# Electron-Labs/eth-lc-plonky2

Measured on AMD Instinct MI355X. Metric: lc_proofs_per_hour, higher is better.
Workload: dtype u64

## Files before the change

eth-lc-plonky2_amd/csrc/kernels_hash.hip:

```cpp
#include "internal.hpp"
#include "poseidon.hpp"

namespace lcp2 {

constexpr int HASH_THREADS = 256;

__global__ __launch_bounds__(HASH_THREADS) void k_poseidon_permute_batch(const u64 *__restrict__ in, u64 *__restrict__ out,
                                                                          size_t count, const u64 *__restrict__ rc) {
  size_t i = (size_t)blockIdx.x * blockDim.x + threadIdx.x;
  if (i >= count) return;
  u64 s[12];
#pragma unroll
  for (int j = 0; j < 12; j++) s[j] = gl_canon(in[i * 12 + j]);
  pos_permute(s, rc);
#pragma unroll
  for (int j = 0; j < 12; j++) out[i * 12 + j] = s[j];
}

__global__ __launch_bounds__(HASH_THREADS) void k_field_op(const u64 *__restrict__ a, const u64 *__restrict__ b, u64 *__restrict__ out,
                                                            size_t count, u32 op) {
  size_t i = (size_t)blockIdx.x * blockDim.x + threadIdx.x;
  if (i >= count) return;
#if defined(__HIP_DEVICE_COMPILE__)
  const u64 x = a[i], y = b ? b[i] : 0;
  u64 r = 0;
  switch (op) {
    case LCP2_FIELD_MUL: r = gl_mul(x, y); break;
    case LCP2_FIELD_POW7: { u32 r0 = (u32)x, r1 = (u32)(x >> 32); pos_sbox_h(r0, r1); r = gl_canon(((u64)r1 << 32) | r0); break; }
    case LCP2_FIELD_ADD: r = gl_add(gl_canon(x), gl_canon(y)); break;
    case LCP2_FIELD_SUB: r = gl_sub(gl_canon(x), gl_canon(y)); break;
    case LCP2_FIELD_CANON: r = gl_canon(x); break;
    case LCP2_FIELD_ADD_LAZY: r = gl_canon(gl_add_nc(x, gl_canon(y))); break;
    case LCP2_FIELD_SUB_LAZY: r = gl_canon(gl_sub_nc(x, gl_canon(y))); break;
    case LCP2_FIELD_SHL + 1: r = gl_shl<12>(gl_canon(x)); break;
    case LCP2_FIELD_SHL + 2: r = gl_shl<24>(gl_canon(x)); break;
    case LCP2_FIELD_SHL + 3: r = gl_shl<36>(gl_canon(x)); break;
    case LCP2_FIELD_SHL + 4: r = gl_shl<48>(gl_canon(x)); break;
    case LCP2_FIELD_SHL + 5: r = gl_shl<60>(gl_canon(x)); break;
    case LCP2_FIELD_SHL + 6: r = gl_shl<72>(gl_canon(x)); break;
    case LCP2_FIELD_SHL + 7: r = gl_shl<84>(gl_canon(x)); break;
    case LCP2_FIELD_SHL + 8: r = gl_canon(gl_shl_nc<32>(x)); break;
    case LCP2_FIELD_SHL + 9: r = gl_canon(gl_mul_u32_nc(x, (u32)y)); break;
  }
  out[i] = r;
#endif
}

__global__ __launch_bounds__(HASH_THREADS, 5) void k_hash_leaves(const u64 *__restrict__ data, u64 leaf_stride, u64 col_stride,
                                                               u32 leaf_len, u64 nleaves, u64 *__restrict__ digests,
                                                               const u64 *__restrict__ rc) {
  u64 i = (u64)blockIdx.x * blockDim.x + threadIdx.x;
  if (i >= nleaves) return;
  const u64 *row = data + i * leaf_stride;
  u64 s[12];
#pragma unroll
  for (int j = 0; j < 12; j++) s[j] = 0;
  if (leaf_len <= 4) {
    for (u32 c = 0; c < leaf_len; c++) s[c] = gl_canon(row[c * col_stride]);
  } else {
    for (u32 c0 = 0; c0 < leaf_len; c0 += 8) {
      if (c0 + 8 <= leaf_len) {
#pragma unroll
        for (int j = 0; j < 8; j++) s[j] = gl_canon(row[(u64)(c0 + j) * col_stride]);
      } else {
#pragma unroll
        for (int j = 0; j < 8; j++)
          if (c0 + j < leaf_len) s[j] = gl_canon(row[(u64)(c0 + j) * col_stride]);
      }
      pos_permute(s, rc);
    }
  }
  ulonglong2 *d = (ulonglong2 *)(digests + 4 * i);
  d[0] = make_ulonglong2(s[0], s[1]);
  d[1] = make_ulonglong2(s[2], s[3]);
}

__global__ __launch_bounds__(HASH_THREADS, 5) void k_hash_leaves_absorb(const u64 *__restrict__ data, u64 col_stride, u32 ncols, u64 nleaves,
                                                                      u64 *__restrict__ state, u32 first, u32 last, u64 *__restrict__ digests,
                                                                      const u64 *__restrict__ rc) {
  u64 i = (u64)blockIdx.x * blockDim.x + threadIdx.x;
  if (i >= nleaves) return;
  const u64 *row = data + i;
  u64 s[12];
#pragma unroll
  for (int j = 0; j < 12; j++) s[j] = first ? 0 : state[(u64)j * nleaves + i];
  for (u32 c0 = 0; c0 < ncols; c0 += 8) {
    if (c0 + 8 <= ncols) {
#pragma unroll
      for (int j = 0; j < 8; j++) s[j] = gl_canon(row[(u64)(c0 + j) * col_stride]);
    } else {
#pragma unroll
      for (int j = 0; j < 8; j++)
        if (c0 + j < ncols) s[j] = gl_canon(row[(u64)(c0 + j) * col_stride]);
    }
    pos_permute(s, rc);
  }
  if (last) {
    ulonglong2 *d = (ulonglong2 *)(digests + 4 * i);
    d[0] = make_ulonglong2(s[0], s[1]);
    d[1] = make_ulonglong2(s[2], s[3]);
  } else {
#pragma unroll
    for (int j = 0; j < 12; j++) state[(u64)j * nleaves + i] = s[j];
  }
}

__global__ __launch_bounds__(HASH_THREADS, 5) void k_hash_ext_leaves(const u64 *__restrict__ p0, const u64 *__restrict__ p1, u32 arity,
                                                                   u64 nleaves, u64 *__restrict__ digests,
                                                                   const u64 *__restrict__ rc) {
  u64 i = (u64)blockIdx.x * blockDim.x + threadIdx.x;
  if (i >= nleaves) return;
  const u64 *a = p0 + i * arity, *b = p1 + i * arity;
  u64 s[12];
#pragma unroll
  for (int j = 0; j < 12; j++) s[j] = 0;
  u32 len = 2 * arity;
  if (len <= 4) {
    for (u32 e = 0; e < arity; e++) { s[2 * e] = a[e]; s[2 * e + 1] = b[e]; }
  } else {
    for (u32 e0 = 0; e0 < arity; e0 += 4) {
#pragma unroll
      for (int j = 0; j < 4; j++)
        if (e0 + j < arity) { s[2 * j] = a[e0 + j]; s[2 * j + 1] = b[e0 + j]; }
      pos_permute(s, rc);
    }
  }
  ulonglong2 *d = (ulonglong2 *)(digests + 4 * i);
  d[0] = make_ulonglong2(s[0], s[1]);
  d[1] = make_ulonglong2(s[2], s[3]);
}

__global__ __launch_bounds__(HASH_THREADS) void k_merkle_level(const u64 *__restrict__ children, u64 *__restrict__ parents,
                                                                u64 nparents, const u64 *__restrict__ rc) {
  u64 i = (u64)blockIdx.x * blockDim.x + threadIdx.x;
  if (i >= nparents) return;
  const ulonglong2 *c = (const ulonglong2 *)(children + 8 * i);
  ulonglong2 c0 = c[0], c1 = c[1], c2 = c[2], c3 = c[3];
  u64 s[12] = {c0.x, c0.y, c1.x, c1.y, c2.x, c2.y, c3.x, c3.y, 0, 0, 0, 0};
  pos_permute(s, rc);
  ulonglong2 *d = (ulonglong2 *)(parents + 4 * i);
  d[0] = make_ulonglong2(s[0], s[1]);
  d[1] = make_ulonglong2(s[2], s[3]);
}

constexpr int COOP_THREADS = 256;
__device__ __forceinline__ void coop_load_rc(u64 *rcs, const u64 *__restrict__ rc) {
  for (u32 i = threadIdx.x; i < POS_ROUNDS * POS_W; i += COOP_THREADS) rcs[i] = rc[i];
  __syncthreads();
}
__global__ __launch_bounds__(COOP_THREADS) void k_merkle_level_coop(const u64 *__restrict__ children, u64 *__restrict__ parents,
                                                                      u64 nparents, const u64 *__restrict__ rc) {
  __shared__ u64 rcs[POS_ROUNDS * POS_W];
  coop_load_rc(rcs, rc);
  const u64 t = (u64)blockIdx.x * COOP_THREADS + threadIdx.x, node = t >> 4;
  const u32 j = (u32)t & 15;
  const bool live = node < nparents;
  const u64 nd = live ? node : 0;
  const u64 v = j < 8 ? children[8 * nd + j] : 0;
  const u64 r = pos_permute_coop(v, j, rcs);
  if (live && j < 4) parents[4 * nd + j] = r;
}
__global__ __launch_bounds__(COOP_THREADS) void k_hash_ext_leaves_coop(const u64 *__restrict__ p0, const u64 *__restrict__ p1, u32 arity,
                                                                         u64 nleaves, u64 *__restrict__ digests, const u64 *__restrict__ rc) {
  __shared__ u64 rcs[POS_ROUNDS * POS_W];
  coop_load_rc(rcs, rc);
  const u64 t = (u64)blockIdx.x * COOP_THREADS + threadIdx.x, leaf = t >> 4;
  const u32 j = (u32)t & 15;
  const bool live = leaf < nleaves;
  const u64 lf = live ? leaf : 0;
  const u64 *src = ((j & 1) ? p1 : p0) + lf * arity + (j >> 1);
  u64 v = 0;
  for (u32 e0 = 0; e0 < arity; e0 += 4) {
    if (j < 8 && e0 + (j >> 1) < arity) v = src[e0];
    v = pos_permute_coop(v, j, rcs);
  }
  if (live && j < 4) digests[4 * lf + j] = v;
}

__device__ __constant__ uint32_t SHA_K[64] = {
    0x428a2f98, 0x71374491, 0xb5c0fbcf, 0xe9b5dba5, 0x3956c25b, 0x59f111f1, 0x923f82a4, 0xab1c5ed5, 0xd807aa98, 0x12835b01,
    0x243185be, 0x550c7dc3, 0x72be5d74, 0x80deb1fe, 0x9bdc06a7, 0xc19bf174, 0xe49b69c1, 0xefbe4786, 0x0fc19dc6, 0x240ca1cc,
    0x2de92c6f, 0x4a7484aa, 0x5cb0a9dc, 0x76f988da, 0x983e5152, 0xa831c66d, 0xb00327c8, 0xbf597fc7, 0xc6e00bf3, 0xd5a79147,
    0x06ca6351, 0x14292967, 0x27b70a85, 0x2e1b2138, 0x4d2c6dfc, 0x53380d13, 0x650a7354, 0x766a0abb, 0x81c2c92e, 0x92722c85,
    0xa2bfe8a1, 0xa81a664b, 0xc24b8b70, 0xc76c51a3, 0xd192e819, 0xd6990624, 0xf40e3585, 0x106aa070, 0x19a4c116, 0x1e376c08,
    0x2748774c, 0x34b0bcb5, 0x391c0cb3, 0x4ed8aa4a, 0x5b9cca4f, 0x682e6ff3, 0x748f82ee, 0x78a5636f, 0x84c87814, 0x8cc70208,
    0x90befffa, 0xa4506ceb, 0xbef9a3f7, 0xc67178f2};

__device__ __forceinline__ uint32_t rotr(uint32_t x, int r) { return __builtin_rotateright32(x, r); }

__device__ __forceinline__ void sha256_compress(uint32_t st[8], uint32_t w[16], uint32_t *trace) {
  uint32_t a = st[0], b = st[1], c = st[2], d = st[3], e = st[4], f = st[5], g = st[6], h = st[7];
#pragma unroll 1
  for (int i = 0; i < 64; i++) {
    uint32_t wi;
    if (i < 16) {
      wi = w[i & 15];
    } else {
      uint32_t w15 = w[(i - 15) & 15], w2 = w[(i - 2) & 15];
      uint32_t s0 = rotr(w15, 7) ^ rotr(w15, 18) ^ (w15 >> 3);
      uint32_t s1 = rotr(w2, 17) ^ rotr(w2, 19) ^ (w2 >> 10);
      wi = w[i & 15] + s0 + w[(i - 7) & 15] + s1;
      w[i & 15] = wi;
      if (trace) trace[i - 16] = wi;
    }
    uint32_t S1 = rotr(e, 6) ^ rotr(e, 11) ^ rotr(e, 25);
    uint32_t ch = (e & f) ^ (~e & g);
    uint32_t t1 = h + S1 + ch + SHA_K[i] + wi;
    uint32_t S0 = rotr(a, 2) ^ rotr(a, 13) ^ rotr(a, 22);
    uint32_t mj = (a & b) ^ (a & c) ^ (b & c);
    uint32_t t2 = S0 + mj;
    h = g; g = f; f = e; e = d + t1; d = c; c = b; b = a; a = t1 + t2;
    if (trace) { trace[48 + 2 * i] = a; trace[48 + 2 * i + 1] = e; }
  }
  st[0] += a; st[1] += b; st[2] += c; st[3] += d; st[4] += e; st[5] += f; st[6] += g; st[7] += h;
}

constexpr int SHA_TRACE_WORDS = 48 + 128;

__global__ __launch_bounds__(64) void k_sha256_level(const uint8_t *__restrict__ children, uint8_t *__restrict__ parents,
                                                      u64 nparents, u64 trees, u64 child_tree_stride, u64 parent_tree_stride,
                                                      uint32_t *__restrict__ trace, u64 trace_tree_stride, u64 trace_hash_offset) {
  u64 gid = (u64)blockIdx.x * blockDim.x + threadIdx.x;
  if (gid >= nparents * trees) return;
  u64 t = gid / nparents, i = gid % nparents;
  const uint32_t *src = (const uint32_t *)(children + t * child_tree_stride + 64 * i);
  uint32_t w[16];
#pragma unroll
  for (int j = 0; j < 16; j++) w[j] = __builtin_bswap32(src[j]);
  uint32_t st[8] = {0x6a09e667, 0xbb67ae85, 0x3c6ef372, 0xa54ff53a, 0x510e527f, 0x9b05688c, 0x1f83d9ab, 0x5be0cd19};
  uint32_t *tr = trace ? trace + t * trace_tree_stride + (trace_hash_offset + i) * 2 * SHA_TRACE_WORDS : nullptr;
  sha256_compress(st, w, tr);
#pragma unroll
  for (int j = 0; j < 16; j++) w[j] = 0;
  w[0] = 0x80000000u; w[15] = 512;
  sha256_compress(st, w, tr ? tr + SHA_TRACE_WORDS : nullptr);
  uint32_t *dst = (uint32_t *)(parents + t * parent_tree_stride + 32 * i);
#pragma unroll
  for (int j = 0; j < 8; j++) dst[j] = __builtin_bswap32(st[j]);
}

__global__ void k_gather_rows(const u64 *__restrict__ data, u64 col_stride, u32 ncols, const u64 *__restrict__ indices, u32 k,
                              u64 *__restrict__ out) {
  u32 q = blockIdx.x;
  if (q >= k) return;
  u64 idx = indices[q];
  for (u32 c = threadIdx.x; c < ncols; c += blockDim.x) out[(u64)q * ncols + c] = data[(u64)c * col_stride + idx];
}
__global__ void k_gather_digests(const u64 *__restrict__ digests, const u64 *__restrict__ level_offsets, u32 nsib,
                                 const u64 *__restrict__ indices, u32 k, u64 *__restrict__ out) {
  u32 q = blockIdx.x;
  if (q >= k) return;
  u64 idx = indices[q];
  for (u32 t = threadIdx.x; t < nsib * 4; t += blockDim.x) {
    u32 l = t >> 2, e = t & 3;
    u64 node = (idx >> l) ^ 1;
    out[((u64)q * nsib + l) * 4 + e] = digests[4 * (level_offsets[l] + node) + e];
  }
}

static inline unsigned blocks_for(u64 n, unsigned threads) { return (unsigned)((n + threads - 1) / threads); }

void launch_poseidon_permute_batch(hipStream_t s, const u64 *in, u64 *out, size_t count, const u64 *rc) {
  if (!count) return;
  hipLaunchKernelGGL(k_poseidon_permute_batch, dim3(blocks_for(count, HASH_THREADS)), dim3(HASH_THREADS), 0, s, in, out, count, rc);
}
void launch_field_op(hipStream_t s, const u64 *a, const u64 *b, u64 *out, size_t count, u32 op) {
  if (!count) return;
  hipLaunchKernelGGL(k_field_op, dim3(blocks_for(count, HASH_THREADS)), dim3(HASH_THREADS), 0, s, a, b, out, count, op);
}
void launch_hash_leaves(hipStream_t s, const u64 *data, u64 leaf_stride, u64 col_stride, u32 leaf_len, u64 nleaves, u64 *digests,
                        const u64 *rc) {
  hipLaunchKernelGGL(k_hash_leaves, dim3(blocks_for(nleaves, HASH_THREADS)), dim3(HASH_THREADS), 0, s, data, leaf_stride, col_stride,
                     leaf_len, nleaves, digests, rc);
}
void launch_hash_leaves_absorb(hipStream_t s, const u64 *data, u64 col_stride, u32 ncols, u64 nleaves, u64 *state, bool first, bool last,
                               u64 *digests, const u64 *rc) {
  hipLaunchKernelGGL(k_hash_leaves_absorb, dim3(blocks_for(nleaves, HASH_THREADS)), dim3(HASH_THREADS), 0, s, data, col_stride, ncols, nleaves,
                     state, first ? 1u : 0u, last ? 1u : 0u, digests, rc);
}
void launch_hash_ext_leaves(hipStream_t s, const u64 *p0, const u64 *p1, u32 arity, u64 nleaves, u64 *digests, const u64 *rc) {
  if (nleaves <= POS_COOP_MAX_NODES && 2 * arity > 4) {
    hipLaunchKernelGGL(k_hash_ext_leaves_coop, dim3(blocks_for(nleaves * 16, COOP_THREADS)), dim3(COOP_THREADS), 0, s, p0, p1, arity, nleaves, digests, rc);
    return;
  }
  hipLaunchKernelGGL(k_hash_ext_leaves, dim3(blocks_for(nleaves, HASH_THREADS)), dim3(HASH_THREADS), 0, s, p0, p1, arity, nleaves,
                     digests, rc);
}
void launch_merkle_level(hipStream_t s, const u64 *children, u64 *parents, u64 nparents, const u64 *rc) {
  if (nparents <= POS_COOP_MAX_NODES) {
    hipLaunchKernelGGL(k_merkle_level_coop, dim3(blocks_for(nparents * 16, COOP_THREADS)), dim3(COOP_THREADS), 0, s, children, parents, nparents, rc);
    return;
  }
  hipLaunchKernelGGL(k_merkle_level, dim3(blocks_for(nparents, HASH_THREADS)), dim3(HASH_THREADS), 0, s, children, parents, nparents, rc);
}
void launch_sha256_level(hipStream_t s, const uint8_t *children, uint8_t *parents, u64 nparents, u64 trees, u64 child_tree_stride,
                         u64 parent_tree_stride, uint32_t *trace, u64 trace_tree_stride, u64 trace_hash_offset) {
  hipLaunchKernelGGL(k_sha256_level, dim3(blocks_for(nparents * trees, 64)), dim3(64), 0, s, children, parents, nparents, trees,
                     child_tree_stride, parent_tree_stride, trace, trace_tree_stride, trace_hash_offset);
}
void launch_gather_rows(hipStream_t s, const u64 *data, u64 col_stride, u32 ncols, const u64 *indices, u32 k, u64 *out) {
  if (!k) return;
  hipLaunchKernelGGL(k_gather_rows, dim3(k), dim3(64), 0, s, data, col_stride, ncols, indices, k, out);
}
void launch_gather_digests(hipStream_t s, const u64 *digests, const u64 *level_offsets, u32 nsib, const u64 *indices, u32 k, u64 *out) {
  if (!k || !nsib) return;
  hipLaunchKernelGGL(k_gather_digests, dim3(k), dim3(64), 0, s, digests, level_offsets, nsib, indices, k, out);
}

}
```

eth-lc-plonky2_amd/csrc/poseidon.hpp:

```cpp
#pragma once
#include <utility>
#include "gl64.hpp"

namespace lcp2 {

constexpr int POS_W = 12;
constexpr int POS_RATE = 8;
constexpr int POS_FULL_HALF = 4;
constexpr int POS_PARTIAL = 22;
constexpr int POS_ROUNDS = 30;

constexpr int POS_GROUP = 3;
constexpr int POS_GROUPS = POS_PARTIAL / POS_GROUP;
constexpr int POS_GROUP_CONSTS = 3 + 11;
constexpr int POS_RC_WORDS = POS_ROUNDS * POS_W + POS_GROUPS * POS_GROUP_CONSTS;

struct PosPartialTables {
  u32 m00, ab, aAb;
  u32 a[11], aA[11], aA2[11], b[11], Ab[11], A2b[11];
  u32 A[11][11], A3[11][11];
};
constexpr PosPartialTables pos_partial_tables() {
  const u32 C[12] = {17, 15, 41, 16, 2, 28, 13, 13, 39, 18, 34, 20};
  PosPartialTables t{};
  u64 M[12][12] = {};
  for (int r = 0; r < 12; r++)
    for (int c = 0; c < 12; c++) M[r][c] = C[(c - r + 12) % 12] + (r == 0 && c == 0 ? 8 : 0);
  u64 A[11][11] = {}, A2[11][11] = {}, A3[11][11] = {}, a[11] = {}, b[11] = {};
  for (int i = 0; i < 11; i++) {
    a[i] = M[0][1 + i];
    b[i] = M[1 + i][0];
    for (int j = 0; j < 11; j++) A[i][j] = M[1 + i][1 + j];
  }
  for (int i = 0; i < 11; i++)
    for (int j = 0; j < 11; j++) {
      u64 acc = 0;
      for (int k = 0; k < 11; k++) acc += A[i][k] * A[k][j];
      A2[i][j] = acc;
    }
  for (int i = 0; i < 11; i++)
    for (int j = 0; j < 11; j++) {
      u64 acc = 0;
      for (int k = 0; k < 11; k++) acc += A2[i][k] * A[k][j];
      A3[i][j] = acc;
    }
  t.m00 = (u32)M[0][0];
  u64 ab = 0, aAb = 0;
  for (int i = 0; i < 11; i++) {
    u64 Ab = 0, A2b = 0, aA = 0, aA2 = 0;
    for (int k = 0; k < 11; k++) { Ab += A[i][k] * b[k]; A2b += A2[i][k] * b[k]; aA += a[k] * A[k][i]; aA2 += a[k] * A2[k][i]; }
    t.a[i] = (u32)a[i]; t.b[i] = (u32)b[i]; t.Ab[i] = (u32)Ab; t.A2b[i] = (u32)A2b; t.aA[i] = (u32)aA; t.aA2[i] = (u32)aA2;
    ab += a[i] * b[i];
    aAb += a[i] * Ab;
    for (int j = 0; j < 11; j++) { t.A[i][j] = (u32)A[i][j]; t.A3[i][j] = (u32)A3[i][j]; }
  }
  t.ab = (u32)ab; t.aAb = (u32)aAb;
  return t;
}
constexpr u32 pos_partial_max_entry() {
  constexpr PosPartialTables t = pos_partial_tables();
  u32 m = t.aAb > t.ab ? t.aAb : t.ab;
  for (int i = 0; i < 11; i++) {
    if (t.A2b[i] > m) m = t.A2b[i];
    if (t.aA2[i] > m) m = t.aA2[i];
    for (int j = 0; j < 11; j++) if (t.A3[i][j] > m) m = t.A3[i][j];
  }
  return m;
}
static_assert(pos_partial_max_entry() < (1u << 22), "grouped partial rounds: a table entry is too large for one multiply-accumulate per half");

LCP2_HD u64 pos_sbox(u64 x) {
  u64 x2 = gl_sqr_nc(x);
  u64 x4 = gl_sqr_nc(x2);
  u64 x3 = gl_mul_nc(x, x2);
  return gl_mul_nc(x3, x4);
}

LCP2_HD void pos_mds(u64 s[12]) {
  const u32 C[12] = {17, 15, 41, 16, 2, 28, 13, 13, 39, 18, 34, 20};
  u32 lo[12], hi[12];
#pragma unroll
  for (int i = 0; i < 12; i++) { lo[i] = (u32)s[i]; hi[i] = (u32)(s[i] >> 32); }
#pragma unroll
  for (int r = 0; r < 12; r++) {
    u64 al = 0, ah = 0;
#pragma unroll
    for (int i = 0; i < 12; i++) {
      al += (u64)lo[(i + r) % 12] * C[i];
      ah += (u64)hi[(i + r) % 12] * C[i];
    }
    if (r == 0) { al += (u64)lo[0] * 8u; ah += (u64)hi[0] * 8u; }
    u64 ah_hi = ah >> 32;
    u64 t = al + ((ah_hi << 32) - ah_hi);
    u64 u = ah << 32;
    u64 v = t + u;
    s[r] = v < t ? v + GL_EPS : v;
  }
}

LCP2_HD void pos_permute_portable(u64 s[12], const u64 *__restrict__ rc) {
  int round = 0;
#pragma unroll 1
  for (int r = 0; r < POS_FULL_HALF; r++, round++) {
#pragma unroll
    for (int i = 0; i < 12; i++) s[i] = pos_sbox(gl_add_nc(s[i], rc[round * 12 + i]));
    pos_mds(s);
  }
#pragma unroll 1
  for (int r = 0; r < POS_PARTIAL; r++, round++) {
#pragma unroll
    for (int i = 0; i < 12; i++) s[i] = gl_add_nc(s[i], rc[round * 12 + i]);
    s[0] = pos_sbox(s[0]);
    pos_mds(s);
  }
#pragma unroll 1
  for (int r = 0; r < POS_FULL_HALF; r++, round++) {
#pragma unroll
    for (int i = 0; i < 12; i++) s[i] = pos_sbox(gl_add_nc(s[i], rc[round * 12 + i]));
    pos_mds(s);
  }
#pragma unroll
  for (int i = 0; i < 12; i++) s[i] = gl_canon(s[i]);
}

inline void pos_extend_round_constants(u64 rc[POS_RC_WORDS]) {
  constexpr PosPartialTables T = pos_partial_tables();
  for (int g = 0; g < POS_GROUPS; g++) {
    const int r = POS_FULL_HALF + POS_GROUP * g;
    const u64 *c1 = rc + 12 * (r + 1), *c2 = rc + 12 * (r + 2), *c3 = rc + 12 * (r + 3);
    u64 *k = rc + POS_ROUNDS * POS_W + POS_GROUP_CONSTS * g;
    u64 v2[11];
    u64 k2 = c2[0], k3 = c3[0];
    for (int i = 0; i < 11; i++) {
      u64 acc = c2[1 + i];
      for (int j = 0; j < 11; j++) acc = gl_add(acc, gl_mul(T.A[i][j], c1[1 + j]));
      v2[i] = acc;
      k2 = gl_add(k2, gl_mul(T.a[i], c1[1 + i]));
    }
    for (int i = 0; i < 11; i++) {
      u64 acc = c3[1 + i];
      for (int j = 0; j < 11; j++) acc = gl_add(acc, gl_mul(T.A[i][j], v2[j]));
      k[3 + i] = acc;
      k3 = gl_add(k3, gl_mul(T.a[i], v2[i]));
    }
    k[0] = c1[0]; k[1] = k2; k[2] = k3;
  }
}

LCP2_HD void pos_permute_grouped_portable(u64 s[12], const u64 *__restrict__ rc) {
  constexpr PosPartialTables T = pos_partial_tables();
  for (int i = 0; i < 12; i++) s[i] = gl_add(gl_canon(s[i]), rc[i]);
  int round = 0;
  for (int r = 0; r < POS_FULL_HALF; r++, round++) {
    for (int i = 0; i < 12; i++) s[i] = gl_canon(pos_sbox(s[i]));
    pos_mds(s);
    for (int i = 0; i < 12; i++) s[i] = gl_add(gl_canon(s[i]), rc[(round + 1) * 12 + i]);
  }
  for (int g = 0; g < POS_GROUPS; g++, round += POS_GROUP) {
    const u64 *k = rc + POS_ROUNDS * POS_W + POS_GROUP_CONSTS * g;
    const u64 *y = s + 1;
    const u64 w0 = gl_canon(pos_sbox(s[0]));
    u64 u1 = gl_add(k[0], gl_mul(T.m00, w0)), u2 = gl_add(k[1], gl_mul(T.ab, w0)), u3 = gl_add(k[2], gl_mul(T.aAb, w0));
    for (int j = 0; j < 11; j++) {
      u1 = gl_add(u1, gl_mul(T.a[j], y[j]));
      u2 = gl_add(u2, gl_mul(T.aA[j], y[j]));
      u3 = gl_add(u3, gl_mul(T.aA2[j], y[j]));
    }
    const u64 w1 = gl_canon(pos_sbox(u1));
    u2 = gl_add(u2, gl_mul(T.m00, w1));
    const u64 w2 = gl_canon(pos_sbox(u2));
    u3 = gl_add(gl_add(u3, gl_mul(T.ab, w1)), gl_mul(T.m00, w2));
    u64 ny[11];
    for (int i = 0; i < 11; i++) {
      u64 acc = gl_add(k[3 + i], gl_add(gl_mul(T.A2b[i], w0), gl_add(gl_mul(T.Ab[i], w1), gl_mul(T.b[i], w2))));
      for (int j = 0; j < 11; j++) acc = gl_add(acc, gl_mul(T.A3[i][j], y[j]));
      ny[i] = acc;
    }
    s[0] = u3;
    for (int i = 0; i < 11; i++) s[1 + i] = ny[i];
  }
  for (; round < POS_FULL_HALF + POS_PARTIAL; round++) {
    s[0] = gl_canon(pos_sbox(s[0]));
    pos_mds(s);
    for (int i = 0; i < 12; i++) s[i] = gl_add(gl_canon(s[i]), rc[(round + 1) * 12 + i]);
  }
  for (int r = 0; r < POS_FULL_HALF; r++, round++) {
    for (int i = 0; i < 12; i++) s[i] = gl_canon(pos_sbox(s[i]));
    pos_mds(s);
    for (int i = 0; i < 12; i++) s[i] = round + 1 < POS_ROUNDS ? gl_add(gl_canon(s[i]), rc[(round + 1) * 12 + i]) : gl_canon(s[i]);
  }
}

#if defined(__HIP_DEVICE_COMPILE__)

__device__ __forceinline__ void pos_sbox_h(u32 &x0, u32 &x1) {
  u32 a0, a1, b0, b1, c0, c1;
  gl_mul_halves(x0, x1, x0, x1, a0, a1);
  gl_mul_halves(a0, a1, a0, a1, b0, b1);
  gl_mul_halves(x0, x1, a0, a1, c0, c1);
  gl_mul_halves(c0, c1, b0, b1, x0, x1);
}

__device__ __forceinline__ void pos_fold_h(u64 al, u64 ah, u32 &r0, u32 &r1) {
  u64 t = (u64)(u32)(ah >> 32) * 0xFFFFFFFFu + al;
  u32 t1 = (u32)(t >> 32), c;
  asm("v_add_co_u32 %0, vcc, %0, %2\n\t"
      "s_nop 1\n\t"
      "v_cndmask_b32_e64 %1, 0, 1, vcc"
      : "+v"(t1), "=&v"(c) : "v"((u32)ah) : "vcc");
  t = ((u64)t1 << 32) | (u32)t;
  u64 q;
  asm("v_mad_u64_u32 %0, vcc, %1, -1, %2" : "=v"(q) : "v"(c), "v"(t) : "vcc");
  r0 = (u32)q;
  r1 = (u32)(q >> 32);
}

#define LCP2_POS_ROW_OPERANDS                                                                                                        \
  : "=&v"(al), "=&v"(ah)                                                                                                             \
  : "v"(l[0]), "v"(l[1]), "v"(l[2]), "v"(l[3]), "v"(l[4]), "v"(l[5]), "v"(l[6]), "v"(l[7]), "v"(l[8]), "v"(l[9]), "v"(l[10]), "v"(l[11]), \
    "v"(h[0]), "v"(h[1]), "v"(h[2]), "v"(h[3]), "v"(h[4]), "v"(h[5]), "v"(h[6]), "v"(h[7]), "v"(h[8]), "v"(h[9]), "v"(h[10]), "v"(h[11]), \
    "s"(klo), "s"(khi)                                                                                                               \
  : "vcc"
template <bool ROW0>
__device__ __forceinline__ void pos_mds_row(const u32 (&l)[12], const u32 (&h)[12], u64 klo , u64 khi, u64 &al, u64 &ah) {
  if constexpr (ROW0) {
    asm(
        "v_mad_u64_u32 %0, vcc, %2, 25, %26\n\t"
        "v_mad_u64_u32 %1, vcc, %14, 25, %27\n\t"
        "v_mad_u64_u32 %0, vcc, %3, 15, %0\n\t"
        "v_mad_u64_u32 %1, vcc, %15, 15, %1\n\t"
        "v_mad_u64_u32 %0, vcc, %4, 41, %0\n\t"
        "v_mad_u64_u32 %1, vcc, %16, 41, %1\n\t"
        "v_mad_u64_u32 %0, vcc, %5, 16, %0\n\t"
        "v_mad_u64_u32 %1, vcc, %17, 16, %1\n\t"
        "v_mad_u64_u32 %0, vcc, %6, 2, %0\n\t"
        "v_mad_u64_u32 %1, vcc, %18, 2, %1\n\t"
        "v_mad_u64_u32 %0, vcc, %7, 28, %0\n\t"
        "v_mad_u64_u32 %1, vcc, %19, 28, %1\n\t"
        "v_mad_u64_u32 %0, vcc, %8, 13, %0\n\t"
        "v_mad_u64_u32 %1, vcc, %20, 13, %1\n\t"
        "v_mad_u64_u32 %0, vcc, %9, 13, %0\n\t"
        "v_mad_u64_u32 %1, vcc, %21, 13, %1\n\t"
        "v_mad_u64_u32 %0, vcc, %10, 39, %0\n\t"
        "v_mad_u64_u32 %1, vcc, %22, 39, %1\n\t"
        "v_mad_u64_u32 %0, vcc, %11, 18, %0\n\t"
        "v_mad_u64_u32 %1, vcc, %23, 18, %1\n\t"
        "v_mad_u64_u32 %0, vcc, %12, 34, %0\n\t"
        "v_mad_u64_u32 %1, vcc, %24, 34, %1\n\t"
        "v_mad_u64_u32 %0, vcc, %13, 20, %0\n\t"
        "v_mad_u64_u32 %1, vcc, %25, 20, %1"
        LCP2_POS_ROW_OPERANDS);
  } else {
    asm(
        "v_mad_u64_u32 %0, vcc, %2, 17, %26\n\t"
        "v_mad_u64_u32 %1, vcc, %14, 17, %27\n\t"
        "v_mad_u64_u32 %0, vcc, %3, 15, %0\n\t"
        "v_mad_u64_u32 %1, vcc, %15, 15, %1\n\t"
        "v_mad_u64_u32 %0, vcc, %4, 41, %0\n\t"
        "v_mad_u64_u32 %1, vcc, %16, 41, %1\n\t"
        "v_mad_u64_u32 %0, vcc, %5, 16, %0\n\t"
        "v_mad_u64_u32 %1, vcc, %17, 16, %1\n\t"
        "v_mad_u64_u32 %0, vcc, %6, 2, %0\n\t"
        "v_mad_u64_u32 %1, vcc, %18, 2, %1\n\t"
        "v_mad_u64_u32 %0, vcc, %7, 28, %0\n\t"
        "v_mad_u64_u32 %1, vcc, %19, 28, %1\n\t"
        "v_mad_u64_u32 %0, vcc, %8, 13, %0\n\t"
        "v_mad_u64_u32 %1, vcc, %20, 13, %1\n\t"
        "v_mad_u64_u32 %0, vcc, %9, 13, %0\n\t"
        "v_mad_u64_u32 %1, vcc, %21, 13, %1\n\t"
        "v_mad_u64_u32 %0, vcc, %10, 39, %0\n\t"
        "v_mad_u64_u32 %1, vcc, %22, 39, %1\n\t"
        "v_mad_u64_u32 %0, vcc, %11, 18, %0\n\t"
        "v_mad_u64_u32 %1, vcc, %23, 18, %1\n\t"
        "v_mad_u64_u32 %0, vcc, %12, 34, %0\n\t"
        "v_mad_u64_u32 %1, vcc, %24, 34, %1\n\t"
        "v_mad_u64_u32 %0, vcc, %13, 20, %0\n\t"
        "v_mad_u64_u32 %1, vcc, %25, 20, %1"
        LCP2_POS_ROW_OPERANDS);
  }
}
#undef LCP2_POS_ROW_OPERANDS

template <u32 C>
__device__ __forceinline__ u64 pos_mac_first(u32 x, u64 k ) {
  static_assert(C <= 64, "inline constants only");
  u64 r;
  asm("v_mad_u64_u32 %0, vcc, %1, %2, %3" : "=v"(r) : "v"(x), "n"(C), "s"(k) : "vcc");
  return r;
}
template <u32 C0>
__device__ __forceinline__ u64 pos_chain_first7(u64 k , u32 x0, const u32 (&x)[6], const u32 (&c)[6]) {
  static_assert(C0 <= 64, "inline constants only");
  u64 acc;
  asm(
      "v_mad_u64_u32 %0, vcc, %1, %8, %15\n\t"
      "v_mad_u64_u32 %0, vcc, %2, %9, %0\n\t"
      "v_mad_u64_u32 %0, vcc, %3, %10, %0\n\t"
      "v_mad_u64_u32 %0, vcc, %4, %11, %0\n\t"
      "v_mad_u64_u32 %0, vcc, %5, %12, %0\n\t"
      "v_mad_u64_u32 %0, vcc, %6, %13, %0\n\t"
      "v_mad_u64_u32 %0, vcc, %7, %14, %0"
      : "=&v"(acc)
      : "v"(x0), "v"(x[0]), "v"(x[1]), "v"(x[2]), "v"(x[3]), "v"(x[4]), "v"(x[5]),
        "n"(C0), "s"(c[0]), "s"(c[1]), "s"(c[2]), "s"(c[3]), "s"(c[4]), "s"(c[5]), "s"(k)
      : "vcc");
  return acc;
}
template <int N>
__device__ __forceinline__ void pos_chain_add(u64 &acc, const u32 (&x)[N], const u32 (&c)[N]) {
  static_assert(N == 6 || N == 7, "six or seven terms");
  if constexpr (N == 6) {
    asm(
      "v_mad_u64_u32 %0, vcc, %1, %7, %0\n\t"
      "v_mad_u64_u32 %0, vcc, %2, %8, %0\n\t"
      "v_mad_u64_u32 %0, vcc, %3, %9, %0\n\t"
      "v_mad_u64_u32 %0, vcc, %4, %10, %0\n\t"
      "v_mad_u64_u32 %0, vcc, %5, %11, %0\n\t"
      "v_mad_u64_u32 %0, vcc, %6, %12, %0"
        : "+v"(acc)
        : "v"(x[0]), "v"(x[1]), "v"(x[2]), "v"(x[3]), "v"(x[4]), "v"(x[5]), "s"(c[0]), "s"(c[1]), "s"(c[2]), "s"(c[3]), "s"(c[4]), "s"(c[5])
        : "vcc");
  } else {
    asm(
      "v_mad_u64_u32 %0, vcc, %1, %8, %0\n\t"
      "v_mad_u64_u32 %0, vcc, %2, %9, %0\n\t"
      "v_mad_u64_u32 %0, vcc, %3, %10, %0\n\t"
      "v_mad_u64_u32 %0, vcc, %4, %11, %0\n\t"
      "v_mad_u64_u32 %0, vcc, %5, %12, %0\n\t"
      "v_mad_u64_u32 %0, vcc, %6, %13, %0\n\t"
      "v_mad_u64_u32 %0, vcc, %7, %14, %0"
        : "+v"(acc)
        : "v"(x[0]), "v"(x[1]), "v"(x[2]), "v"(x[3]), "v"(x[4]), "v"(x[5]), "v"(x[6]),
          "s"(c[0]), "s"(c[1]), "s"(c[2]), "s"(c[3]), "s"(c[4]), "s"(c[5]), "s"(c[6])
        : "vcc");
  }
}
template <class F, int... I>
__device__ __forceinline__ void pos_static_for_impl(F &&f, std::integer_sequence<int, I...>) { (f(std::integral_constant<int, I>{}), ...); }
template <int N, class F>
__device__ __forceinline__ void pos_static_for(F &&f) { pos_static_for_impl(f, std::make_integer_sequence<int, N>{}); }

__device__ __forceinline__ void pos_mds_h(u32 lo[12], u32 hi[12], const u64 *__restrict__ add) {
  u32 nl[12], nh[12];
#pragma unroll
  for (int r = 0; r < 12; r++) {
    const u64 k = add ? add[r] : 0;
    u32 l[12], h[12];
#pragma unroll
    for (int i = 0; i < 12; i++) { l[i] = lo[(i + r) % 12]; h[i] = hi[(i + r) % 12]; }
    u64 al, ah;
    if (r == 0) pos_mds_row<true>(l, h, (u64)(u32)k, k >> 32, al, ah);
    else pos_mds_row<false>(l, h, (u64)(u32)k, k >> 32, al, ah);
    pos_fold_h(al, ah, nl[r], nh[r]);
  }
#pragma unroll
  for (int r = 0; r < 12; r++) { lo[r] = nl[r]; hi[r] = nh[r]; }
}

template <class Consts , class NextW>
__device__ __forceinline__ void pos_partial3_core(u32 lo[12], u32 hi[12], Consts kc, NextW next_w) {
  constexpr PosPartialTables T = pos_partial_tables();
  u32 w0l = lo[0], w0h = hi[0], w1l, w1h, w2l, w2h;
  pos_sbox_h(w0l, w0h);
  {
    const u64 c = kc[0];
    u32 l[12], h[12];
    l[0] = w0l; h[0] = w0h;
#pragma unroll
    for (int j = 1; j < 12; j++) { l[j] = lo[j]; h[j] = hi[j]; }
    u64 al, ah;
    pos_mds_row<true>(l, h, (u64)(u32)c, c >> 32, al, ah);
    pos_fold_h(al, ah, w1l, w1h);
    next_w(1, w1l, w1h);
  }
  auto row = [&](auto c0, u64 k, u32 xl0, u32 xh0, const u32 (&ca)[6], const u32 (&cb5)[5], u32 cw0, u32 cw1, bool has_w1, u32 &rl, u32 &rh) {
    constexpr u32 C0 = decltype(c0)::value;
    const u32 xa_l[6] = {lo[1], lo[2], lo[3], lo[4], lo[5], lo[6]}, xa_h[6] = {hi[1], hi[2], hi[3], hi[4], hi[5], hi[6]};
    u64 al = pos_chain_first7<C0>((u64)(u32)k, xl0, xa_l, ca), ah = pos_chain_first7<C0>(k >> 32, xh0, xa_h, ca);
    if (has_w1) {
      const u32 xb_l[7] = {lo[7], lo[8], lo[9], lo[10], lo[11], w0l, w1l}, xb_h[7] = {hi[7], hi[8], hi[9], hi[10], hi[11], w0h, w1h};
      const u32 cb[7] = {cb5[0], cb5[1], cb5[2], cb5[3], cb5[4], cw0, cw1};
      pos_chain_add<7>(al, xb_l, cb);
      pos_chain_add<7>(ah, xb_h, cb);
    } else {
      const u32 xb_l[6] = {lo[7], lo[8], lo[9], lo[10], lo[11], w0l}, xb_h[6] = {hi[7], hi[8], hi[9], hi[10], hi[11], w0h};
      const u32 cb[6] = {cb5[0], cb5[1], cb5[2], cb5[3], cb5[4], cw0};
      pos_chain_add<6>(al, xb_l, cb);
      pos_chain_add<6>(ah, xb_h, cb);
    }
    pos_fold_h(al, ah, rl, rh);
  };
  {
    const u32 ca[6] = {T.aA[0], T.aA[1], T.aA[2], T.aA[3], T.aA[4], T.aA[5]}, cb5[5] = {T.aA[6], T.aA[7], T.aA[8], T.aA[9], T.aA[10]};
    row(std::integral_constant<u32, T.m00>{}, kc[1], w1l, w1h, ca, cb5, T.ab, 0, false, w2l, w2h);
    next_w(2, w2l, w2h);
  }
  u32 nl[12], nh[12];
  {
    const u32 ca[6] = {T.aA2[0], T.aA2[1], T.aA2[2], T.aA2[3], T.aA2[4], T.aA2[5]}, cb5[5] = {T.aA2[6], T.aA2[7], T.aA2[8], T.aA2[9], T.aA2[10]};
    row(std::integral_constant<u32, T.m00>{}, kc[2], w2l, w2h, ca, cb5, T.aAb, T.ab, true, nl[0], nh[0]);
  }
  pos_static_for<11>([&](auto ii) {
    constexpr int i = decltype(ii)::value;
    const u32 ca[6] = {T.A3[i][0], T.A3[i][1], T.A3[i][2], T.A3[i][3], T.A3[i][4], T.A3[i][5]},
              cb5[5] = {T.A3[i][6], T.A3[i][7], T.A3[i][8], T.A3[i][9], T.A3[i][10]};
    row(std::integral_constant<u32, T.b[i]>{}, kc[3 + i], w2l, w2h, ca, cb5, T.A2b[i], T.Ab[i], true, nl[1 + i], nh[1 + i]);
  });
#pragma unroll
  for (int r = 0; r < 12; r++) { lo[r] = nl[r]; hi[r] = nh[r]; }
}
__device__ __forceinline__ void pos_partial3_h(u32 lo[12], u32 hi[12], const u64 *__restrict__ kc) {
  pos_partial3_core(lo, hi, kc, [&](int, u32 &ul, u32 &uh) { pos_sbox_h(ul, uh); });
}

__device__ __forceinline__ void pos_permute_gfx950(u64 s[12], const u64 *__restrict__ rc) {
  u32 lo[12], hi[12];
#pragma unroll
  for (int i = 0; i < 12; i++) { u64 v = gl_add_nc(s[i], rc[i]); lo[i] = (u32)v; hi[i] = (u32)(v >> 32); }
  int round = 0;
#pragma unroll 1
  for (int r = 0; r < POS_FULL_HALF; r++, round++) {
#pragma unroll
    for (int i = 0; i < 12; i++) pos_sbox_h(lo[i], hi[i]);
    pos_mds_h(lo, hi, rc + (round + 1) * 12);
  }
#pragma unroll 1
  for (int g = 0; g < POS_GROUPS; g++, round += POS_GROUP) pos_partial3_h(lo, hi, rc + POS_ROUNDS * POS_W + POS_GROUP_CONSTS * g);
#pragma unroll 1
  for (; round < POS_FULL_HALF + POS_PARTIAL; round++) {
    pos_sbox_h(lo[0], hi[0]);
    pos_mds_h(lo, hi, rc + (round + 1) * 12);
  }
#pragma unroll 1
  for (int r = 0; r < POS_FULL_HALF - 1; r++, round++) {
#pragma unroll
    for (int i = 0; i < 12; i++) pos_sbox_h(lo[i], hi[i]);
    pos_mds_h(lo, hi, rc + (round + 1) * 12);
  }
#pragma unroll
  for (int i = 0; i < 12; i++) pos_sbox_h(lo[i], hi[i]);
  pos_mds_h(lo, hi, nullptr);
#pragma unroll
  for (int i = 0; i < 12; i++) s[i] = gl_canon(((u64)hi[i] << 32) | lo[i]);
}

template <class SboxIn>
__device__ __forceinline__ u64 pos_permute_coop_hooked(u64 v, u32 j, const u64 *__restrict__ rc , SboxIn sbox_in) {
  const u32 C[12] = {17, 15, 41, 16, 2, 28, 13, 13, 39, 18, 34, 20};
  const u32 lane = __lane_id(), jj = j < 12 ? j : 0, base = lane - j;
  u32 src[12];
#pragma unroll
  for (int i = 0; i < 12; i++) src[i] = (base + (jj + i >= 12 ? jj + i - 12 : jj + i)) << 2;
  v = gl_add_nc(v, rc[jj]);
  u32 lo = (u32)v, hi = (u32)(v >> 32);
  auto mds = [&](u64 add) {
    u64 al = (u32)add, ah = add >> 32;
    al += (u64)lo * C[0];
    ah += (u64)hi * C[0];
#pragma unroll
    for (int i = 1; i < 12; i++) {
      const u32 vl = (u32)__builtin_amdgcn_ds_bpermute((int)src[i], (int)lo), vh = (u32)__builtin_amdgcn_ds_bpermute((int)src[i], (int)hi);
      al += (u64)vl * C[i];
      ah += (u64)vh * C[i];
    }
    if (j == 0) { al += (u64)lo * 8u; ah += (u64)hi * 8u; }
    pos_fold_h(al, ah, lo, hi);
  };
  int round = 0;
#pragma unroll 1
  for (int r = 0; r < POS_FULL_HALF; r++, round++) {
    const u64 next = rc[(round + 1) * 12 + jj];
    sbox_in(round, lo, hi);
    pos_sbox_h(lo, hi);
    mds(next);
  }
#pragma unroll 1
  for (int r = 0; r < POS_PARTIAL; r++, round++) {
    const u64 next = rc[(round + 1) * 12 + jj];
    sbox_in(round, lo, hi);
    u32 s0 = lo, s1 = hi;
    pos_sbox_h(s0, s1);
    if (j == 0) { lo = s0; hi = s1; }
    mds(next);
  }
#pragma unroll 1
  for (int r = 0; r < POS_FULL_HALF; r++, round++) {
    const u64 next = round + 1 < POS_ROUNDS ? rc[(round + 1) * 12 + jj] : 0;
    sbox_in(round, lo, hi);
    pos_sbox_h(lo, hi);
    mds(next);
  }
  return gl_canon(((u64)hi << 32) | lo);
}
__device__ __forceinline__ u64 pos_permute_coop(u64 v, u32 j, const u64 *__restrict__ rc) {
  return pos_permute_coop_hooked(v, j, rc, [](int, u32, u32) {});
}
#elif defined(__HIPCC__)
__device__ u64 pos_permute_coop(u64 v, u32 j, const u64 *__restrict__ rc);
template <class SboxIn>
__device__ __forceinline__ u64 pos_permute_coop_hooked(u64, u32, const u64 *__restrict__, SboxIn) { return 0; }
#endif
constexpr u32 POS_COOP_MAX_NODES = 4096;

LCP2_HD void pos_permute(u64 s[12], const u64 *__restrict__ rc) {
#if defined(__HIP_DEVICE_COMPILE__)
  pos_permute_gfx950(s, rc);
#else
  pos_permute_portable(s, rc);
#endif
}

inline void pos_derive_round_constants(u64 out[POS_ROUNDS * POS_W]) {
  auto rotl = [](u32 x, int r) { return (u32)((x << r) | (x >> (32 - r))); };
  u32 key[8];
  u64 st = 0;
  for (int i = 0; i < 8; i++) {
    st = st * 6364136223846793005ull + 11634580027462260723ull;
    u32 xs = (u32)(((st >> 18) ^ st) >> 27);
    int rot = (int)(st >> 59);
    key[i] = rot ? (u32)((xs >> rot) | (xs << (32 - rot))) : xs;
  }
  u32 blk[16];
  int pos = 16, got = 0;
  u64 ctr = 0;
  while (got < POS_ROUNDS * POS_W) {
    u32 w[2];
    for (int k = 0; k < 2; k++) {
      if (pos == 16) {
        u32 in[16] = {0x61707865u, 0x3320646eu, 0x79622d32u, 0x6b206574u};
        for (int i = 0; i < 8; i++) in[4 + i] = key[i];
        in[12] = (u32)ctr; in[13] = (u32)(ctr >> 32); in[14] = 0; in[15] = 0;
        ctr++;
        u32 x[16];
        for (int i = 0; i < 16; i++) x[i] = in[i];
        auto qr = [&](int a, int b, int c, int d) {
          x[a] += x[b]; x[d] ^= x[a]; x[d] = rotl(x[d], 16);
          x[c] += x[d]; x[b] ^= x[c]; x[b] = rotl(x[b], 12);
          x[a] += x[b]; x[d] ^= x[a]; x[d] = rotl(x[d], 8);
          x[c] += x[d]; x[b] ^= x[c]; x[b] = rotl(x[b], 7);
        };
        for (int r = 0; r < 4; r++) {
          qr(0, 4, 8, 12); qr(1, 5, 9, 13); qr(2, 6, 10, 14); qr(3, 7, 11, 15);
          qr(0, 5, 10, 15); qr(1, 6, 11, 12); qr(2, 7, 8, 13); qr(3, 4, 9, 14);
        }
        for (int i = 0; i < 16; i++) blk[i] = x[i] + in[i];
        pos = 0;
      }
      w[k] = blk[pos++];
    }
    u64 v = (u64)w[0] | ((u64)w[1] << 32);
    unsigned __int128 m = (unsigned __int128)v * GL_P;
    if ((u64)m <= 0xFFFFFFFF00000000ull) out[got++] = (u64)(m >> 64);
  }
}

}
```

Baseline: 8728.

## Skip unused MDS outputs and zero-capacity first-round sboxes in Poseidon sponges

Splits the Poseidon permutation into a body and a masked final MDS tail, so that sponge absorption computes only the output lanes it needs: the four digest lanes at the end, or the four capacity lanes when the rate lanes will be overwritten. When the capacity starts at zero, the first-round S-boxes for the capacity lanes are replaced by precomputed constants appended to the round-constant table. Leaf, ext-leaf and Merkle-level kernels are routed through a shared sponge-absorb helper. This removes redundant field arithmetic per permutation, at the cost of more code paths, a larger constant table, and gl_canon no longer being applied to the input words the old leaf kernels loaded.

After: 8853 (median of 6 runs). +1.4%, better.

```diff
diff --git a/eth-lc-plonky2_amd/csrc/kernels_hash.hip b/eth-lc-plonky2_amd/csrc/kernels_hash.hip
--- a/eth-lc-plonky2_amd/csrc/kernels_hash.hip
+++ b/eth-lc-plonky2_amd/csrc/kernels_hash.hip
@@ -56,19 +56,11 @@
 #pragma unroll
   for (int j = 0; j < 12; j++) s[j] = 0;
   if (leaf_len <= 4) {
-    for (u32 c = 0; c < leaf_len; c++) s[c] = gl_canon(row[c * col_stride]);
+#pragma unroll
+    for (int c = 0; c < 4; c++)
+      if (c < (int)leaf_len) s[c] = gl_canon(row[c * col_stride]);
   } else {
-    for (u32 c0 = 0; c0 < leaf_len; c0 += 8) {
-      if (c0 + 8 <= leaf_len) {
-#pragma unroll
-        for (int j = 0; j < 8; j++) s[j] = gl_canon(row[(u64)(c0 + j) * col_stride]);
-      } else {
-#pragma unroll
-        for (int j = 0; j < 8; j++)
-          if (c0 + j < leaf_len) s[j] = gl_canon(row[(u64)(c0 + j) * col_stride]);
-      }
-      pos_permute(s, rc);
-    }
+    pos_sponge_absorb(s, leaf_len, rc, true, true, [&](u32 c0, int j) { return row[(u64)(c0 + j) * col_stride]; });
   }
   ulonglong2 *d = (ulonglong2 *)(digests + 4 * i);
   d[0] = make_ulonglong2(s[0], s[1]);
@@ -84,17 +76,7 @@
   u64 s[12];
 #pragma unroll
   for (int j = 0; j < 12; j++) s[j] = first ? 0 : state[(u64)j * nleaves + i];
-  for (u32 c0 = 0; c0 < ncols; c0 += 8) {
-    if (c0 + 8 <= ncols) {
-#pragma unroll
-      for (int j = 0; j < 8; j++) s[j] = gl_canon(row[(u64)(c0 + j) * col_stride]);
-    } else {
-#pragma unroll
-      for (int j = 0; j < 8; j++)
-        if (c0 + j < ncols) s[j] = gl_canon(row[(u64)(c0 + j) * col_stride]);
-    }
-    pos_permute(s, rc);
-  }
+  pos_sponge_absorb(s, ncols, rc, first != 0, last != 0, [&](u32 c0, int j) { return row[(u64)(c0 + j) * col_stride]; });
   if (last) {
     ulonglong2 *d = (ulonglong2 *)(digests + 4 * i);
     d[0] = make_ulonglong2(s[0], s[1]);
@@ -116,14 +98,11 @@
   for (int j = 0; j < 12; j++) s[j] = 0;
   u32 len = 2 * arity;
   if (len <= 4) {
-    for (u32 e = 0; e < arity; e++) { s[2 * e] = a[e]; s[2 * e + 1] = b[e]; }
+#pragma unroll
+    for (int e = 0; e < 2; e++)
+      if (e < (int)arity) { s[2 * e] = a[e]; s[2 * e + 1] = b[e]; }
   } else {
-    for (u32 e0 = 0; e0 < arity; e0 += 4) {
-#pragma unroll
-      for (int j = 0; j < 4; j++)
-        if (e0 + j < arity) { s[2 * j] = a[e0 + j]; s[2 * j + 1] = b[e0 + j]; }
-      pos_permute(s, rc);
-    }
+    pos_sponge_absorb(s, len, rc, true, true, [&](u32 c0, int j) { return (j & 1) ? b[(c0 >> 1) + (j >> 1)] : a[(c0 >> 1) + (j >> 1)]; });
   }
   ulonglong2 *d = (ulonglong2 *)(digests + 4 * i);
   d[0] = make_ulonglong2(s[0], s[1]);
@@ -137,7 +116,8 @@
   const ulonglong2 *c = (const ulonglong2 *)(children + 8 * i);
   ulonglong2 c0 = c[0], c1 = c[1], c2 = c[2], c3 = c[3];
   u64 s[12] = {c0.x, c0.y, c1.x, c1.y, c2.x, c2.y, c3.x, c3.y, 0, 0, 0, 0};
-  pos_permute(s, rc);
+  pos_permute_body(s, rc, true);
+  pos_permute_tail<POS_TAIL_FINAL>(s);
   ulonglong2 *d = (ulonglong2 *)(parents + 4 * i);
   d[0] = make_ulonglong2(s[0], s[1]);
   d[1] = make_ulonglong2(s[2], s[3]);
diff --git a/eth-lc-plonky2_amd/csrc/poseidon.hpp b/eth-lc-plonky2_amd/csrc/poseidon.hpp
--- a/eth-lc-plonky2_amd/csrc/poseidon.hpp
+++ b/eth-lc-plonky2_amd/csrc/poseidon.hpp
@@ -13,7 +13,8 @@
 constexpr int POS_GROUP = 3;
 constexpr int POS_GROUPS = POS_PARTIAL / POS_GROUP;
 constexpr int POS_GROUP_CONSTS = 3 + 11;
-constexpr int POS_RC_WORDS = POS_ROUNDS * POS_W + POS_GROUPS * POS_GROUP_CONSTS;
+constexpr int POS_RC_ZERO_CAP = POS_ROUNDS * POS_W + POS_GROUPS * POS_GROUP_CONSTS;
+constexpr int POS_RC_WORDS = POS_RC_ZERO_CAP + 4;
 
 struct PosPartialTables {
   u32 m00, ab, aAb;
@@ -145,14 +146,20 @@
     }
     k[0] = c1[0]; k[1] = k2; k[2] = k3;
   }
-}
-
-LCP2_HD void pos_permute_grouped_portable(u64 s[12], const u64 *__restrict__ rc) {
+  for (int i = 0; i < POS_W - POS_RATE; i++) rc[POS_RC_ZERO_CAP + i] = gl_canon(pos_sbox(rc[POS_RATE + i]));
+}
+
+constexpr u32 POS_TAIL_FINAL = 0x00F;
+constexpr u32 POS_TAIL_CAPACITY = 0xF00;
+constexpr u32 POS_TAIL_FULL = 0xFFF;
+
+constexpr u64 POS_POISON = 0xFFFFFFFF5EEDDEADull;
+LCP2_HD void pos_permute_body_portable(u64 s[12], const u64 *__restrict__ rc, bool zero_cap) {
   constexpr PosPartialTables T = pos_partial_tables();
   for (int i = 0; i < 12; i++) s[i] = gl_add(gl_canon(s[i]), rc[i]);
   int round = 0;
   for (int r = 0; r < POS_FULL_HALF; r++, round++) {
-    for (int i = 0; i < 12; i++) s[i] = gl_canon(pos_sbox(s[i]));
+    for (int i = 0; i < 12; i++) s[i] = zero_cap && r == 0 && i >= POS_RATE ? rc[POS_RC_ZERO_CAP + i - POS_RATE] : gl_canon(pos_sbox(s[i]));
     pos_mds(s);
     for (int i = 0; i < 12; i++) s[i] = gl_add(gl_canon(s[i]), rc[(round + 1) * 12 + i]);
   }
@@ -184,11 +191,29 @@
     pos_mds(s);
     for (int i = 0; i < 12; i++) s[i] = gl_add(gl_canon(s[i]), rc[(round + 1) * 12 + i]);
   }
-  for (int r = 0; r < POS_FULL_HALF; r++, round++) {
+  for (int r = 0; r < POS_FULL_HALF - 1; r++, round++) {
     for (int i = 0; i < 12; i++) s[i] = gl_canon(pos_sbox(s[i]));
     pos_mds(s);
-    for (int i = 0; i < 12; i++) s[i] = round + 1 < POS_ROUNDS ? gl_add(gl_canon(s[i]), rc[(round + 1) * 12 + i]) : gl_canon(s[i]);
-  }
+    for (int i = 0; i < 12; i++) s[i] = gl_add(gl_canon(s[i]), rc[(round + 1) * 12 + i]);
+  }
+  for (int i = 0; i < 12; i++) s[i] = gl_canon(pos_sbox(s[i]));
+}
+template <u32 MASK>
+LCP2_HD void pos_mds_tail_portable(u64 s[12]) {
+  u64 t[12];
+  for (int i = 0; i < 12; i++) t[i] = s[i];
+  pos_mds(t);
+  for (int r = 0; r < 12; r++) {
+    if ((MASK >> r) & 1) s[r] = gl_canon(t[r]);
+#if !defined(__HIPCC__)
+    else s[r] = POS_POISON;
+#endif
+  }
+}
+
+LCP2_HD void pos_permute_grouped_portable(u64 s[12], const u64 *__restrict__ rc) {
+  pos_permute_body_portable(s, rc, false);
+  pos_mds_tail_portable<POS_TAIL_FULL>(s);
 }
 
 #if defined(__HIP_DEVICE_COMPILE__)
@@ -413,7 +438,7 @@
   pos_partial3_core(lo, hi, kc, [&](int, u32 &ul, u32 &uh) { pos_sbox_h(ul, uh); });
 }
 
-__device__ __forceinline__ void pos_permute_gfx950(u64 s[12], const u64 *__restrict__ rc) {
+__device__ __forceinline__ void pos_permute_body_gfx950(u64 s[12], const u64 *__restrict__ rc, bool zero_cap) {
   u32 lo[12], hi[12];
 #pragma unroll
   for (int i = 0; i < 12; i++) { u64 v = gl_add_nc(s[i], rc[i]); lo[i] = (u32)v; hi[i] = (u32)(v >> 32); }
@@ -421,7 +446,14 @@
 #pragma unroll 1
   for (int r = 0; r < POS_FULL_HALF; r++, round++) {
 #pragma unroll
-    for (int i = 0; i < 12; i++) pos_sbox_h(lo[i], hi[i]);
+    for (int i = 0; i < POS_RATE; i++) pos_sbox_h(lo[i], hi[i]);
+    if (zero_cap && r == 0) {
+#pragma unroll
+      for (int i = POS_RATE; i < 12; i++) { const u64 k = rc[POS_RC_ZERO_CAP + i - POS_RATE]; lo[i] = (u32)k; hi[i] = (u32)(k >> 32); }
+    } else {
+#pragma unroll
+      for (int i = POS_RATE; i < 12; i++) pos_sbox_h(lo[i], hi[i]);
+    }
     pos_mds_h(lo, hi, rc + (round + 1) * 12);
   }
 #pragma unroll 1
@@ -438,10 +470,29 @@
     pos_mds_h(lo, hi, rc + (round + 1) * 12);
   }
 #pragma unroll
-  for (int i = 0; i < 12; i++) pos_sbox_h(lo[i], hi[i]);
-  pos_mds_h(lo, hi, nullptr);
-#pragma unroll
-  for (int i = 0; i < 12; i++) s[i] = gl_canon(((u64)hi[i] << 32) | lo[i]);
+  for (int i = 0; i < 12; i++) { pos_sbox_h(lo[i], hi[i]); s[i] = ((u64)hi[i] << 32) | lo[i]; }
+}
+template <u32 MASK>
+__device__ __forceinline__ void pos_mds_tail(u64 s[12]) {
+  u32 lo[12], hi[12];
+#pragma unroll
+  for (int i = 0; i < 12; i++) { lo[i] = (u32)s[i]; hi[i] = (u32)(s[i] >> 32); }
+  pos_static_for<12>([&](auto rr) {
+    constexpr int r = decltype(rr)::value;
+    if constexpr ((MASK >> r) & 1) {
+      u32 l[12], h[12], nl, nh;
+#pragma unroll
+      for (int i = 0; i < 12; i++) { l[i] = lo[(i + r) % 12]; h[i] = hi[(i + r) % 12]; }
+      u64 al, ah;
+      pos_mds_row<r == 0>(l, h, 0, 0, al, ah);
+      pos_fold_h(al, ah, nl, nh);
+      s[r] = gl_canon(((u64)nh << 32) | nl);
+    }
+  });
+}
+__device__ __forceinline__ void pos_permute_gfx950(u64 s[12], const u64 *__restrict__ rc) {
+  pos_permute_body_gfx950(s, rc, false);
+  pos_mds_tail<POS_TAIL_FULL>(s);
 }
 
 template <class SboxIn>
@@ -508,6 +559,46 @@
 #else
   pos_permute_portable(s, rc);
 #endif
+}
+LCP2_HD void pos_permute_body(u64 s[12], const u64 *__restrict__ rc, bool zero_cap) {
+#if defined(__HIP_DEVICE_COMPILE__)
+  pos_permute_body_gfx950(s, rc, zero_cap);
+#else
+  pos_permute_body_portable(s, rc, zero_cap);
+#endif
+}
+template <u32 MASK>
+LCP2_HD void pos_permute_tail(u64 s[12]) {
+#if defined(__HIP_DEVICE_COMPILE__)
+  pos_mds_tail<MASK>(s);
+#else
+  pos_mds_tail_portable<MASK>(s);
+#endif
+}
+
+template <class Load>
+LCP2_HD void pos_sponge_absorb(u64 s[12], u32 len, const u64 *__restrict__ rc, bool zero_cap, bool finish, Load load) {
+#pragma unroll
+  for (int j = 0; j < POS_RATE; j++)
+    if (len >= POS_RATE || j < (int)len) s[j] = load(0u, j);
+  for (u32 c0 = POS_RATE;; c0 += POS_RATE) {
+    pos_permute_body(s, rc, zero_cap && c0 == POS_RATE);
+    if (c0 >= len && finish) {
+      pos_permute_tail<POS_TAIL_FINAL>(s);
+      return;
+    }
+    if (c0 + POS_RATE <= len) {
+      pos_permute_tail<POS_TAIL_CAPACITY>(s);
+#pragma unroll
+      for (int j = 0; j < POS_RATE; j++) s[j] = load(c0, j);
+    } else {
+      pos_permute_tail<POS_TAIL_FULL>(s);
+#pragma unroll
+      for (int j = 0; j < POS_RATE; j++)
+        if (c0 + j < len) s[j] = load(c0, j);
+      if (c0 >= len) return;
+    }
+  }
 }
 
 inline void pos_derive_round_constants(u64 out[POS_ROUNDS * POS_W]) {
```
